# MartinPippel/DAmar

Hardware: AMD Instinct MI355X
Metric: aligned base-pairs/sec (daligner block-vs-block) (higher is better)
Workload: dtype int32

## Files before the change

damar_amd/csrc/kernels/kernels.h:

```cpp
#ifndef DAMAR_KERNELS_H
#define DAMAR_KERNELS_H

#include "dev_common.h"

size_t damar_scan_workspace_bytes(u64 n);
void   damar_exclusive_scan_u32(const u32 *in, u32 *out, u64 n, void *work, u64 *total_dev, hipStream_t st);
#define DAMAR_SCAN_TILE 4096
void   damar_tile_offsets_u32(const u32 *in, u64 n, void *work, u64 *total_dev, hipStream_t st);
void   damar_scan_tile_counts(u32 *tcount, u32 ntiles, u64 *total_dev, hipStream_t st);
size_t damar_sort_workspace_bytes(u64 n);
void   damar_sort_set_threads(int threads);
const u32 *damar_sort_error_word(const void *work);
int    damar_radix_sort_keys_u64(u64 *k0, u64 *k1, u64 n, int lobit, int hibit, void *work, hipStream_t st);
void   damar_radix_sort_split_u64(u64 *k0, u64 *k1, u64 n, int lobit, int hibit, u32 *ohi, u32 *olo, void *work,
                                  hipStream_t st);
int    damar_radix_sort_u32(u32 *k0, u32 *v0, u32 *k1, u32 *v1, u64 n, int nbits, void *work, hipStream_t st);
int    damar_radix_sort_keys_u32(u32 *k0, u32 *k1, u64 n, int nbits, void *work, hipStream_t st);
int    damar_radix_sort_u64(u64 *k0, u32 *v0, u64 *k1, u32 *v1, u64 n, int nbits, void *work, hipStream_t st);

enum { DAMAR_PILE_COVER = 0, DAMAR_PILE_REPEAT = 1, DAMAR_PILE_TANDEM = 2 };
#define DAMAR_PILE_ERR_RANGE 1u
typedef struct
{
  const long long *pile_off;
  const int *pile_aread, *abpos, *aepos, *bbpos, *bepos, *bread, *flags, *read_len, *read_flags;
  u32   npiles;
  int   mode, pbits;
  int   min_len, inc_identity, inccov, enter, leave, merge_dist;
  u64  *keys;
  u32  *kept;
  const u32 *koff;
  u64  *bases;
  int  *active;
  int  *rb, *re, *rc;
  int  *out;
  u32  *count;
  u64  *stats;
  u32  *err;
} PileArgs;
void damar_launch_pile_events(const PileArgs *a, hipStream_t st);
void damar_launch_pile_sweep(const PileArgs *a, hipStream_t st);
void damar_launch_pile_gather(const int *out, const u32 *koff, const u32 *count, const u32 *doff, u32 npiles, int *dst, hipStream_t st);

typedef struct
{ const u8  *bases;
  const u32 *pk;
  u32        rbias;
  const u32 *boff;
  const u32 *coarse;
  u32        nreads;
  u32        total;
  int        maxlen;
  int        rpbits;
  const u32 *moff;
  const int *mdat;
} DevBlock;

#define SEED_PRIO_VAR(name, dflt) static __device__ int name = dflt;  static int name##_host = dflt;
#define SEED_PRIO(name)     do { if (name) __builtin_amdgcn_s_setprio(3); } while (0)
#define SEED_PRIO_SETTER(fn, name) \
  void fn(int on) { if (on != name##_host) { HIP_CHECK(hipMemcpyToSymbol(HIP_SYMBOL(name), &on, sizeof(int)));  name##_host = on; } }

#define COARSE_SHIFT 9
#define PK_PAD 4

#ifdef __HIPCC__
__device__ __forceinline__ u32 read_of_pos(const DevBlock &b, u32 p)
{ u32 r = b.coarse[p >> COARSE_SHIFT];
  while (b.boff[r + 1] <= p)
    r += 1;
  return r;
}
__device__ __forceinline__ void pos_decode(const DevBlock &b, u32 v, u32 *r, u32 *x)
{ if (b.rpbits)
    { *r = v >> b.rpbits;
      *x = v & ((1u << b.rpbits) - 1u);
    }
  else
    { const u32 rr = read_of_pos(b, v);
      *r = rr;
      *x = v - b.boff[rr];
    }
}
__device__ __forceinline__ u32 pos_encode(const DevBlock &b, u32 r, u32 x, u32 p)
{ return b.rpbits ? ((r << b.rpbits) | x) : p; }
#endif

long long damar_pack_words(u32 total);
void damar_launch_pack_bases(const u8 *bases, u32 total, u32 *pk, hipStream_t st);
void damar_launch_unpack_bps(const u8 *raw, const u32 *foff, const DevBlock *blk, int comp, u8 *bases, hipStream_t st);

void damar_preload_index(void);  void damar_preload_scan(void);  void damar_preload_sort(void);
void damar_preload_merge(void);  void damar_preload_report(void);
void damar_sort_set_prio(int on);
void damar_merge_set_prio(int on);
void damar_index_set_prio(int on);
void damar_launch_kmer_tuples(const DevBlock *blk, int kmer, u32 nkmers, void *codes, int wide, u32 *pos, hipStream_t st);
void damar_launch_mask_flags(const DevBlock *blk, int kmer, const u32 *pos, u32 n, u32 *keep, hipStream_t st);
void damar_launch_biased_tuples(const DevBlock *blk, int kmer, const int *logbase, void *codes, int wide, u32 *pos,
                                u32 *keep, hipStream_t st);
void damar_launch_suppress_flags(const void *codes, int wide, u32 n, int suppress, u32 *keep, hipStream_t st);
void damar_launch_compact_pairs(const void *k, int wide, const u32 *v, const u32 *keep, const u32 *off, u32 n,
                                void *ko, u32 *vo, hipStream_t st);

void damar_launch_tandem_links(const DevBlock *blk, int kmer, const void *codes, int wide, const u32 *pos, u32 n,
                               int *dist, hipStream_t st);

typedef struct
{ const void *acode;  const u32 *apos;  u32 alen;
  const void *bcode;  const u32 *bpos;  u32 blen;
  int  wide;
  int  kbits;
  int  self, comp, identity;
  u32  limit;
  DevBlock ablk, bblk;
  int  pbits, abits;
  int  dbits;
  u32  b_lo, b_hi;
} MergeArgs;

typedef struct { u32 b0, b1, ja, ia;
                 u32 sh, pad[3]; } MergeTile;

size_t damar_merge_workspace_bytes(u32 alen);
u32   *damar_merge_tile_counts(void *work, u32 alen);
u32    damar_merge_tiles(u32 alen);
void   damar_launch_merge_count(const MergeArgs *m, void *work, unsigned long long *gram, u32 ngram, hipStream_t st);
void damar_launch_merge_emit(const MergeArgs *m, void *work, u64 nhits, u64 *keys, u32 *vals, u32 *pid, hipStream_t st);
void damar_launch_merge_bread_hist(const MergeArgs *m, void *work, unsigned long long *hist, hipStream_t st);
void damar_launch_merge_range(const MergeArgs *m, void *work, hipStream_t st);
void damar_launch_pair_heads_ids(const u32 *pids, u64 nhits, u64 off, u64 gtotal, int abits, int minhit, int nshift,
                                 u64 *send, u64 *bits, void *scan_work, u64 *total_dev, u32 *heads, hipStream_t st);
void damar_launch_pair_bitmap(const u32 *pids, const u32 *heads, u32 nheads, int abits, u32 b_lo, u32 b_hi, u32 *bitmap,
                              hipStream_t st);
void damar_launch_seed_cut_count(const u64 *keys, u64 nhits, int pbits, const u32 *bitmap, u32 *tcount, u64 *total_dev,
                                 hipStream_t st);
void damar_launch_seed_cut_scatter(const u64 *keys, const u32 *vals, u64 nhits, int pbits, const u32 *bitmap,
                                   const u32 *toff, u64 *okeys, u32 *ovals, hipStream_t st);
// ... 174 lines not shown
```

damar_amd/csrc/kernels/kmer_index.hip:

```cpp
#include "dev_common.h"
#include "kernels.h"

SEED_PRIO_VAR(g_index_prio, 0)
SEED_PRIO_SETTER(damar_index_set_prio, g_index_prio)


template <typename CodeT, bool PACK>
__global__ __launch_bounds__(256)
void kmer_tuples(DevBlock blk, int kmer, u32 nkmers, CodeT *__restrict__ codes, u32 *__restrict__ pos)
{ SEED_PRIO(g_index_prio);
  const u32 p = blockIdx.x * 256u + threadIdx.x;
  if (p >= blk.total)
    return;
  const u32 r = read_of_pos(blk, p), b0 = blk.boff[r];
  if (p - b0 < (u32) (kmer - 1) || p + 1 == blk.boff[r + 1])
    return;
  const u32 i = p - (r + 1) * (u32) kmer + 1;
  if (i >= nkmers)
    return;
  CodeT c = 0;
  if (PACK)
    {
      const u32 f = p - (u32) (kmer - 1), wq = f >> 4, o = (f & 15) << 1;
      u64 win = ((u64) blk.pk[wq + 1] << 32) | (u64) blk.pk[wq];
      win >>= o;
      u64 r = __brevll(win);
      r = ((r >> 1) & 0x5555555555555555ull) | ((r & 0x5555555555555555ull) << 1);
      c = (CodeT) (r >> (64 - 2 * kmer));
    }
  else
    { const u8 *s = blk.bases + (p - (u32) (kmer - 1));
      for (int j = 0; j < kmer; j++)
        c = (CodeT) (c << 2) | (CodeT) s[j];
    }
  const u32 pw = pos_encode(blk, r, p - b0, p);
  if (PACK)
    codes[i] = (CodeT) ((u64) c << 32) | (CodeT) pw;
  else
    { codes[i] = c;
      pos[i]   = pw;
    }
}

void damar_launch_kmer_tuples(const DevBlock *blk, int kmer, u32 nkmers, void *codes, int wide, u32 *pos, hipStream_t st)
{ if (nkmers == 0)
    return;
  if (wide)
    hipLaunchKernelGGL((kmer_tuples<u64, false>), dim3((blk->total + 255) / 256), dim3(256), 0, st, *blk, kmer, nkmers, (u64 *) codes, pos);
  else if (pos == NULL)
    hipLaunchKernelGGL((kmer_tuples<u64, true>), dim3((blk->total + 255) / 256), dim3(256), 0, st, *blk, kmer, nkmers, (u64 *) codes, pos);
  else
    hipLaunchKernelGGL((kmer_tuples<u32, false>), dim3((blk->total + 255) / 256), dim3(256), 0, st, *blk, kmer, nkmers, (u32 *) codes, pos);
}

__global__ __launch_bounds__(256)
void mask_flags(DevBlock blk, int kmer, const u32 *__restrict__ pos, u32 n, u32 *__restrict__ keep)
{ u32 i = blockIdx.x * 256u + threadIdx.x;
  if (i >= n)
    return;
  u32 r, x;
  pos_decode(blk, pos[i], &r, &x);
  const int e = (int) x, s = e - (kmer - 1);
  u32 lo = blk.moff[r] >> 1, hi = blk.moff[r + 1] >> 1;
  const u32 end = hi;
  while (lo < hi)
    { const u32 mid = (lo + hi) >> 1;
      if (blk.mdat[2 * mid + 1] > s) hi = mid; else lo = mid + 1;
    }
  keep[i] = (lo < end && blk.mdat[2 * lo] <= e) ? 0u : 1u;
}

void damar_launch_mask_flags(const DevBlock *blk, int kmer, const u32 *pos, u32 n, u32 *keep, hipStream_t st)
{ if (n == 0)
    return;
  hipLaunchKernelGGL(mask_flags, dim3((n + 255) / 256), dim3(256), 0, st, *blk, kmer, pos, n, keep);
}

template <typename CodeT>
__global__ __launch_bounds__(64)
void biased_tuples(DevBlock blk, int kmer, int lb0, int lb1, int lb2, int lb3,
                   CodeT *__restrict__ codes, u32 *__restrict__ pos, u32 *__restrict__ keep)
{ const u32 r = blockIdx.x * 64u + threadIdx.x;
// ... 237 lines not shown
```

damar_amd/csrc/kernels/radix_sort.hip:

```cpp
#include <atomic>
#include <type_traits>
#include "dev_common.h"
#include "kernels.h"

SEED_PRIO_VAR(g_sort_prio, 1)
SEED_PRIO_SETTER(damar_sort_set_prio, g_sort_prio)

#ifndef OS_THREADS
#define OS_THREADS 1024
#endif
#ifndef OS_MINW
#define OS_MINW    4
#endif
#ifndef OS_RANK_LDS
#define OS_RANK_LDS 1
#endif
#define OS_MINTILE (256 * 8)
#define OS_MAXPASS 8

#define OH_ITEMS   16

#define LB_COUNT   1u
#define LB_PREFIX  2u
#define LB_SPINS   (1u << 24)
#ifndef LB_AHEAD
#define LB_AHEAD   8
#endif

#define WS_HIST    256
#define WS_CTR     (256 + OS_MAXPASS * 256 * 4)
#define WS_LB      16384

template <typename GT> __device__ __forceinline__ GT lb_load(const GT *p)
{ return __hip_atomic_load(p, __ATOMIC_RELAXED, __HIP_MEMORY_SCOPE_AGENT); }
template <typename GT> __device__ __forceinline__ void lb_store(GT *p, GT v)
{ __hip_atomic_store(p, v, __ATOMIC_RELAXED, __HIP_MEMORY_SCOPE_AGENT); }

__device__ __forceinline__ u32 os_scan256(u32 v, u32 *lds4)
{ const int l = lane_id(), w = threadIdx.x >> 6;
  const u32 inc = (u32) wave_incl_scan_i((int) v);
  if (l == 63 && w < 4) lds4[w] = inc;
  __syncthreads();
  u32 base = 0;
  for (int i = 0; i < 4; i++)
    if (i < w) base += lds4[i];
  __syncthreads();
  return base + inc - v;
}


#define OH_THREADS 1024
#define OH_BINMAX  61440

template <typename KeyT>
__global__ __launch_bounds__(OH_THREADS)
void onesweep_hist(const KeyT *__restrict__ keys, u64 n, int lobit, int npass, u64 dsh ,
                   u64 dwd , u32 *__restrict__ ghist, uint4 *__restrict__ clr, u64 clr16)
{ extern __shared__ u32 sh[];
  constexpr u32 nthr = OH_THREADS;
  const int nw = npass * 128 * 32;
  for (int j = threadIdx.x; j < nw; j += nthr)
    sh[j] = 0;
  __syncthreads();
  const u32 c = threadIdx.x & 31u;
  const u64 ntile = (n + (u64) nthr * OH_ITEMS - 1) / ((u64) nthr * OH_ITEMS);
  for (u64 t = blockIdx.x; t < ntile; t += gridDim.x)
    { const u64 base = t * ((u64) nthr * OH_ITEMS);
      KeyT k[OH_ITEMS];
#pragma unroll
      for (int r = 0; r < OH_ITEMS; r++)
        { const u64 i = base + (u64) r * nthr + threadIdx.x;
          k[r] = (i < n) ? keys[i] : (KeyT) 0;
        }
#pragma unroll
      for (int r = 0; r < OH_ITEMS; r++)
        { const u64 i = base + (u64) r * nthr + threadIdx.x;
          if (i < n)
            { const KeyT x = k[r] >> lobit;
              for (int p = 0; p < npass; p++)
                { const u32 d = (u32) (x >> (int) ((dsh >> (8 * p)) & 0xffu)) & (u32) ((dwd >> (8 * p)) & 0xffu);
                  atomicAdd(&sh[((u32) p << 12) + ((d >> 1) << 5) + c], 1u << ((d & 1u) << 4));
                }
            }
        }
    }
  __syncthreads();
  for (int j = threadIdx.x; j < npass * 256; j += nthr)
    { const u32 pl = (u32) j >> 8, d = (u32) j & 0xffu, sft = (d & 1u) << 4;
      u32 sum = 0;
#pragma unroll 8
      for (u32 q = 0; q < 32; q++)
        sum += (sh[(pl << 12) + ((d >> 1) << 5) + ((q + threadIdx.x) & 31u)] >> sft) & 0xffffu;
      if (sum)
        atomicAdd(&ghist[j], sum);
    }
  const uint4 z = make_uint4(0, 0, 0, 0);
  for (u64 i = (u64) blockIdx.x * nthr + threadIdx.x; i < clr16; i += (u64) gridDim.x * nthr)
    clr[i] = z;
}

#define OH_COPIES  8
template <typename KeyT>
__global__ __launch_bounds__(256)
void onesweep_hist8(const KeyT *__restrict__ keys, u64 n, int lobit, int npass, u64 dsh ,
                   u64 dwd , u32 *__restrict__ ghist, uint4 *__restrict__ clr, u64 clr16)
{ SEED_PRIO(g_sort_prio);
  extern __shared__ u32 sh[];
  const int nb = npass * 256 * OH_COPIES;
  for (int j = threadIdx.x; j < nb; j += 256)
    sh[j] = 0;
  __syncthreads();
  const u32 c = threadIdx.x & (OH_COPIES - 1);
  const u64 ntile = (n + 256 * OH_ITEMS - 1) / (256 * OH_ITEMS);
  for (u64 t = blockIdx.x; t < ntile; t += gridDim.x)
    { const u64 base = t * (256 * OH_ITEMS);
      KeyT k[OH_ITEMS];
#pragma unroll
      for (int r = 0; r < OH_ITEMS; r++)
        { const u64 i = base + (u64) r * 256 + threadIdx.x;
          k[r] = (i < n) ? keys[i] : (KeyT) 0;
        }
#pragma unroll
      for (int r = 0; r < OH_ITEMS; r++)
        { const u64 i = base + (u64) r * 256 + threadIdx.x;
          if (i < n)
            { const KeyT x = k[r] >> lobit;
              for (int p = 0; p < npass; p++)
                { const u32 d = (u32) (x >> (int) ((dsh >> (8 * p)) & 0xffu)) & (u32) ((dwd >> (8 * p)) & 0xffu);
                  atomicAdd(&sh[(((u32) p << 8) + d) * OH_COPIES + c], 1u);
                }
            }
        }
    }
  __syncthreads();
  for (int j = threadIdx.x; j < npass * 256; j += 256)
    { u32 s = 0;
#pragma unroll
      for (int q = 0; q < OH_COPIES; q++)
        s += sh[j * OH_COPIES + q];
      if (s)
        atomicAdd(&ghist[j], s);
    }
  const uint4 z = make_uint4(0, 0, 0, 0);
  for (u64 i = (u64) blockIdx.x * 256 + threadIdx.x; i < clr16; i += (u64) gridDim.x * 256)
    clr[i] = z;
}


template <typename KeyT, typename GT, bool HV, bool SPLIT, int TH, int IT>
__global__ __launch_bounds__(TH, (IT <= 8 ? 8 : OS_MINW))
void onesweep_pass(const KeyT *__restrict__ kin, const u32 *__restrict__ vin, KeyT *__restrict__ kout,
                   u32 *__restrict__ vout, u32 *__restrict__ ohi, u64 n, int shift, u32 mask,
                   const u32 *__restrict__ ghist, GT *__restrict__ lb, GT *__restrict__ lbclear,
                   u32 *__restrict__ ctr, u32 *__restrict__ err)
{ SEED_PRIO(g_sort_prio);
  constexpr int OS_TILE = TH * IT, OS_WAVES = TH / 64, OS_WSPAN = 64 * IT;
  __shared__ __attribute__((aligned(16))) KeyT skey[OS_TILE];
  u32 *const sval = (u32 *) skey;
  typedef typename std::conditional<(OS_WAVES > 8), u16, u32>::type CntT;
  __shared__ CntT cnt[OS_WAVES][256];
  __shared__ u32  dstart[256];
  __shared__ u32  gadj[256];
  __shared__ u32  lds4[4];
  __shared__ u32  s_tile;
  constexpr int SH = (int) sizeof(GT) * 8 - 2;
  constexpr GT  VM = (((GT) 1) << SH) - 1;

  const int l = lane_id(), w = threadIdx.x >> 6;
  if (threadIdx.x == 0)
    s_tile = atomicAdd(ctr, 1u);
  for (int i = 0; i < OS_WAVES; i++)
    if (threadIdx.x < 256)
      cnt[i][threadIdx.x] = 0;
#if OS_RANK_LDS
  static_assert((size_t) OS_TILE * sizeof(KeyT) >= (size_t) OS_WAVES * 256 * sizeof(u64), "the rank words do not fit the stage");
  for (int i = threadIdx.x; i < OS_WAVES * 256; i += TH)
    ((u64 *) skey)[i] = 0;
#endif
  __syncthreads();
  const u32 tile  = (u32) __builtin_amdgcn_readfirstlane((int) s_tile);
  const u64 tbase = (u64) tile * OS_TILE;
  const u32 have = (n - tbase < (u64) OS_TILE) ? (u32) (n - tbase) : (u32) OS_TILE;
  const u32 t0 = (u32) w * OS_WSPAN + (u32) l;
  const KeyT *const tin = kin + tbase;

  KeyT key[IT];
  u32  rnk[IT];
#pragma unroll
  for (int r = 0; r < IT; r++)
    { const u32 ti = t0 + (u32) r * 64;
      key[r] = tin[ti < have ? ti : have - 1];
    }
#if OS_RANK_LDS
  u64 *const wmask = (u64 *) skey + (u32) w * 256u;
  const u64 lanebit = 1ull << l;
#pragma unroll
  for (int r = 0; r < IT; r++)
    { const bool ok = t0 + (u32) r * 64 < have;
      const u32  d  = (u32) (key[r] >> shift) & mask;
      if (ok)
        __hip_atomic_fetch_or(&wmask[d], lanebit, __ATOMIC_RELAXED, __HIP_MEMORY_SCOPE_WAVEFRONT);
      __builtin_amdgcn_fence(__ATOMIC_SEQ_CST, "wavefront");
      const u64 peers  = __hip_atomic_load(&wmask[d], __ATOMIC_RELAXED, __HIP_MEMORY_SCOPE_WAVEFRONT);
      const u32 before = cnt[w][d];
      __builtin_amdgcn_fence(__ATOMIC_SEQ_CST, "wavefront");
      const u32 mine   = __builtin_amdgcn_mbcnt_hi((u32) (peers >> 32), __builtin_amdgcn_mbcnt_lo((u32) peers, 0u));
      rnk[r] = before + mine;
      if (ok && mine == 0)
        { cnt[w][d] = (CntT) (before + (u32) __popcll(peers));
          __hip_atomic_store(&wmask[d], 0ull, __ATOMIC_RELAXED, __HIP_MEMORY_SCOPE_WAVEFRONT);
        }
      __builtin_amdgcn_fence(__ATOMIC_SEQ_CST, "wavefront");
    }
#else
#pragma unroll
  for (int r = 0; r < IT; r++)
    { const bool ok = t0 + (u32) r * 64 < have;
      const u32  d  = (u32) (key[r] >> shift) & mask;
      const u64 okm = __ballot(ok);
      u32 plo = (u32) okm, phi = (u32) (okm >> 32);
#pragma unroll
      for (int b = 0; b < 8; b++)
        { const int t  = ((int) (d << (31 - b))) >> 31;
          const u64 nm = ~__ballot(t < 0);
          plo &= (u32) nm ^ (u32) t;
          phi &= (u32) (nm >> 32) ^ (u32) t;
        }
      const u32 before = cnt[w][d];
      const u32 mine   = __builtin_amdgcn_mbcnt_hi(phi, __builtin_amdgcn_mbcnt_lo(plo, 0u));
      rnk[r] = before + mine;
      if (ok && mine == 0)
        cnt[w][d] = (CntT) (before + (u32) __popc(plo) + (u32) __popc(phi));
    }
#endif
  __syncthreads();

  u32 tot = 0;
  if (threadIdx.x < 256)
    { u32 run = 0;
#pragma unroll
      for (int i = 0; i < OS_WAVES; i++)
        { const u32 c = cnt[i][threadIdx.x];
          cnt[i][threadIdx.x] = (CntT) run;
          run += c;
// ... 77 lines not shown
        { const KeyT k = skey[i];
          const u32  d = (u32) (k >> shift) & mask;
          const u32  g = gadj[d] + i;
          if (HV) gdst[q] = g;
          if (SPLIT)
            { ohi[g]  = (u32) ((u64) k >> 32);
              vout[g] = (u32) k;
            }
          else
            kout[g] = k;
        }
    }
  if (HV)
    { const u32 *const tvin = vin + tbase;
      __syncthreads();
#pragma unroll
      for (int r = 0; r < IT; r++)
        { const u32 ti = t0 + (u32) r * 64;
          if (ti < have)
            sval[rnk[r]] = tvin[ti];
        }
      __syncthreads();
#pragma unroll
      for (int q = 0; q < IT; q++)
        { const u32 i = threadIdx.x + (u32) q * TH;
          if (i < have)
            vout[gdst[q]] = sval[i];
        }
    }
}


static int G_sort_threads = 0;

void damar_sort_set_threads(int threads) { G_sort_threads = (threads == 256 || threads == 512) ? threads : 1024; }

static int sort_threads(void)
{ if (G_sort_threads == 0)
    { const char *e = getenv("DAMAR_SORT_THREADS");
      damar_sort_set_threads(e ? atoi(e) : OS_THREADS);
    }
  return G_sort_threads;
}

size_t damar_sort_workspace_bytes(u64 n)
{ const u64 ntiles = (n + OS_MINTILE - 1) / OS_MINTILE;
  return (size_t) WS_LB + 2 * (((size_t) ntiles * 256 * sizeof(u64) + 255) & ~(size_t) 255) + 256;
}

const u32 *damar_sort_error_word(const void *work) { return (const u32 *) work; }

template <typename KeyT, typename GT, bool HV, int TH, int IT>
static void onesweep_passes(KeyT *k0, u32 *v0, KeyT *k1, u32 *v1, u64 n, int lobit, int hibit, u32 *ohi, u32 *olo,
                            char *ws, hipStream_t st)
{ constexpr int OS_TILE = TH * IT;
  const u32 ntiles = (u32) ((n + OS_TILE - 1) / OS_TILE);
  const int npass  = (hibit - lobit + 7) / 8;
  int dshift[OS_MAXPASS], dwidth[OS_MAXPASS];
  u64 dsh = 0, dwd = 0;
  { const int bits = hibit - lobit, base = bits / npass, extra = bits % npass;
    int at = 0;
    static int even = -1;
    if (even < 0)
      { const char *e = getenv("DAMAR_SORT_EVEN");
        even = e ? atoi(e) : 1;
      }
    for (int p = 0; p < npass; p++)
      { dshift[p] = at;
        dwidth[p] = even ? base + (p < extra ? 1 : 0) : (p < npass - 1 ? 8 : bits - 8 * (npass - 1));
        at += dwidth[p];
        dsh |= (u64) dshift[p] << (8 * p);
        dwd |= (u64) ((1u << dwidth[p]) - 1u) << (8 * p);
      }
  }
  const size_t region = ((size_t) ntiles * 256 * sizeof(GT) + 255) & ~(size_t) 255;
  u32 *err = (u32 *) ws, *ghist = (u32 *) (ws + WS_HIST), *ctr = (u32 *) (ws + WS_CTR);
  GT  *lbr[2] = { (GT *) (ws + WS_LB), (GT *) (ws + WS_LB + region) };
  HIP_CHECK(hipMemsetAsync(ws, 0, WS_LB, st));
  if (sort_threads() >= 512)
    { const u64 nt = (n + (u64) OH_THREADS * OH_ITEMS - 1) / ((u64) OH_THREADS * OH_ITEMS);
      const u64 maxit = OH_BINMAX / ((OH_THREADS / 32) * OH_ITEMS);
      u64 grid = nt < 512 ? nt : 512;
      if ((nt + grid - 1) / grid > maxit)
        grid = (nt + maxit - 1) / maxit;
      const size_t lds = (size_t) npass * 128 * 32 * sizeof(u32);
      {
        static std::atomic<unsigned long long> big_lds(0ull);
        int dev = 0;
        HIP_CHECK(hipGetDevice(&dev));
        const unsigned long long bit = 1ull << (dev & 63);
        if (!(big_lds.load(std::memory_order_acquire) & bit))
          { HIP_CHECK(hipFuncSetAttribute((const void *) onesweep_hist<u32>, hipFuncAttributeMaxDynamicSharedMemorySize, 8 * 16384));
            HIP_CHECK(hipFuncSetAttribute((const void *) onesweep_hist<u64>, hipFuncAttributeMaxDynamicSharedMemorySize, 8 * 16384));
            big_lds.fetch_or(bit, std::memory_order_release);
          }
      }
      hipLaunchKernelGGL(onesweep_hist<KeyT>, dim3((u32) grid), dim3(OH_THREADS), lds, st,
                         k0, n, lobit, npass, dsh, dwd, ghist, (uint4 *) lbr[0], (u64) (region / 16));
      HIP_CHECK(hipGetLastError());
    }
  else
    { const u64 nt = (n + 256 * OH_ITEMS - 1) / (256 * OH_ITEMS);
      const u32 grid = (u32) (nt < 2048 ? nt : 2048);
      hipLaunchKernelGGL(onesweep_hist8<KeyT>, dim3(grid), dim3(256), (size_t) npass * 256 * OH_COPIES * sizeof(u32), st,
                         k0, n, lobit, npass, dsh, dwd, ghist, (uint4 *) lbr[0], (u64) (region / 16));
    }
  for (int p = 0; p < npass; p++)
    { const int  side = p & 1;
      const bool last = (p == npass - 1);
      KeyT *ki = side ? k1 : k0, *ko = side ? k0 : k1;
      u32  *vi = side ? v1 : v0, *vo = side ? v0 : v1;
      const u32 mask = (1u << dwidth[p]) - 1u;
      if (last && ohi != NULL)
        hipLaunchKernelGGL((onesweep_pass<KeyT, GT, false, true, TH, IT>), dim3(ntiles), dim3(TH), 0, st,
                           ki, (const u32 *) NULL, (KeyT *) NULL, olo, ohi, n, lobit + dshift[p], mask,
                           ghist + 256 * p, lbr[side], lbr[side ^ 1], ctr + p, err);
      else
        hipLaunchKernelGGL((onesweep_pass<KeyT, GT, HV, false, TH, IT>), dim3(ntiles), dim3(TH), 0, st,
                           ki, vi, ko, vo, (u32 *) NULL, n, lobit + dshift[p], mask,
                           ghist + 256 * p, lbr[side], lbr[side ^ 1], ctr + p, err);
    }
}

template <typename KeyT, bool HV>
static int onesweep_impl(KeyT *k0, u32 *v0, KeyT *k1, u32 *v1, u64 n, int lobit, int hibit, u32 *ohi, u32 *olo,
                         void *work, hipStream_t st)
{ const int npass = (hibit - lobit + 7) / 8;
  if (n == 0 || npass <= 0)
    return 0;
  if (npass > OS_MAXPASS || n >= 0xfffffff0ull)
    { fprintf(stderr, "damar: internal error, radix sort of %llu items on %d bits\n", (unsigned long long) n, hibit - lobit);
      fflush(NULL);
      _exit(1);
    }
  const int shape = sort_threads();
  static int lb64 = -1;
  if (lb64 < 0)
    lb64 = getenv("DAMAR_SORT_LB64") != NULL;
  if (n < (1ull << 30) && !lb64)
    { if (shape == 1024)     onesweep_passes<KeyT, u32, HV, 1024, 8>(k0, v0, k1, v1, n, lobit, hibit, ohi, olo, (char *) work, st);
      else if (shape == 512) onesweep_passes<KeyT, u32, HV, 512, 16>(k0, v0, k1, v1, n, lobit, hibit, ohi, olo, (char *) work, st);
      else              onesweep_passes<KeyT, u32, HV, 256, 16>(k0, v0, k1, v1, n, lobit, hibit, ohi, olo, (char *) work, st);
    }
  else
    onesweep_passes<KeyT, u64, HV, 256, 16>(k0, v0, k1, v1, n, lobit, hibit, ohi, olo, (char *) work, st);
  return npass & 1;
}

int damar_radix_sort_u32(u32 *k0, u32 *v0, u32 *k1, u32 *v1, u64 n, int nbits, void *work, hipStream_t st)
{ return onesweep_impl<u32, true>(k0, v0, k1, v1, n, 0, nbits, NULL, NULL, work, st); }

int damar_radix_sort_keys_u32(u32 *k0, u32 *k1, u64 n, int nbits, void *work, hipStream_t st)
{ return onesweep_impl<u32, false>(k0, NULL, k1, NULL, n, 0, nbits, NULL, NULL, work, st); }

int damar_radix_sort_u64(u64 *k0, u32 *v0, u64 *k1, u32 *v1, u64 n, int nbits, void *work, hipStream_t st)
{ return onesweep_impl<u64, true>(k0, v0, k1, v1, n, 0, nbits, NULL, NULL, work, st); }

int damar_radix_sort_keys_u64(u64 *k0, u64 *k1, u64 n, int lobit, int hibit, void *work, hipStream_t st)
{ return onesweep_impl<u64, false>(k0, NULL, k1, NULL, n, lobit, hibit, NULL, NULL, work, st); }

void damar_radix_sort_split_u64(u64 *k0, u64 *k1, u64 n, int lobit, int hibit, u32 *ohi, u32 *olo, void *work,
                                hipStream_t st)
{ onesweep_impl<u64, false>(k0, NULL, k1, NULL, n, lobit, hibit, ohi, olo, work, st); }

void damar_preload_sort(void)
{ hipFuncAttributes fa;
  (void) hipFuncGetAttributes(&fa, (const void *) onesweep_hist<u64>);
}
```

damar_amd/csrc/shim.hip:

```cpp
#include <algorithm>
#include <vector>
#include <deque>
#include <string>
#include <thread>
#include <atomic>
#include <mutex>
#include <condition_variable>
#include <functional>
#include <string.h>
#include <unistd.h>

#include "kernels/dev_common.h"
#include <ctype.h>
#include "kernels/kernels.h"

extern "C" {
#include "damar_filter.h"
#include "damar_hip.h"
#include "host/damar_host.h"
}

#define MAXGRAM 10000

static void die(void)
// ... 596 lines not shown
  HIP_CHECK(hipFree(b->coarse));
  free(b);
}


struct damar_dev_index
{ size_t codes_bytes, pos_bytes;
  damar_dev_block *blk;
  int   own_block;
  void *codes;
  u32  *pos;
  u32   n;
  int   kbits, wide;
};

static u32 *H_serr = NULL;
static int  H_nserr = 0;
static void sort_verify(void)
{ for (int i = 0; i < H_nserr; i++)
    if (H_serr[i] != 0)
      { fprintf(stderr, "damar: FATAL: the radix sort's look-back timed out\n");
        die();
      }
  H_nserr = 0;
}
static void sort_check(const void *sw)
{ if (H_serr == NULL)
    HIP_CHECK(hipHostMalloc((void **) &H_serr, 64 * sizeof(u32), hipHostMallocDefault));
  if (H_nserr == 64)
    { HIP_CHECK(hipStreamSynchronize(G_st));
      sort_verify();
    }
  HIP_CHECK(hipMemcpyAsync(&H_serr[H_nserr++], damar_sort_error_word(sw), sizeof(u32), hipMemcpyDeviceToHost, G_st));
}

static bool overlap_on(void);
static bool corun_on(void);
static void pick_sort_shape(void)
{ static int forced = -1;
  if (forced < 0)
    { const char *e = getenv("DAMAR_SORT_THREADS");
      forced = e ? atoi(e) : 0;
    }
  damar_sort_set_threads(forced ? forced : 1024);
}

static int ilog2_ceil(u64 n)
{ int b = 0;
  while ((1ull << b) < n)
    b += 1;
  return b;
}

static int  B_have = 0, B_log[4];

extern "C" void damar_bias_reset(void) { B_have = 0; }

static damar_dev_index *index_build_k(damar_dev_block *blk, int own_block, int *len, int K, int suppress, int use_bias)
{ ensure_init();
  pick_sort_shape();
  if (K > 32)
    { fprintf(stderr, "damar: FATAL: -k%d: a k-mer code holds at most 32 bases\n", K);
      die();
    }
  if (blk->nreads > 0 && blk->minlen < K)
    { fprintf(stderr, "[ERROR] - daligner: Block contains reads < %dbp long !  Run DBsplit.\n", K);
      die();
    }
  int64 nk64 = (int64) blk->d.total - (int64) K * blk->nreads;
  if (nk64 <= 0)
    { *len = 0;
      if (own_block)
        damar_block_free(blk);
      return NULL;
    }
  u32 nk = (u32) nk64;
  const int kbits = 2 * K;
  const int wide = K > 16;
  const size_t cs = wide ? sizeof(u64) : sizeof(u32);
  const bool masked = blk->d.moff != NULL;
  const bool biased = use_bias != 0;
  if (biased && !B_have)
    { const double scale = -10000. / log(4.);
      for (int i = 0; i < 4; i++)
        B_log[i] = (int) ceil(scale * log((double) blk->freq[i]));
      B_have = 1;
    }
  const u32 cap = biased ? blk->d.total : nk;
  const int npass = (kbits + 7) / 8;
  damar_dev_index *ix = (damar_dev_index *) calloc(1, sizeof(damar_dev_index));
  ix->blk = blk;  ix->own_block = own_block;  ix->kbits = kbits;  ix->wide = wide;
  if (wide)
    { ix->codes = dpool_get(cs * (size_t) cap, &ix->codes_bytes);
      ix->pos   = (u32 *) dpool_get(sizeof(u32) * (size_t) cap, &ix->pos_bytes);
    }
  else
    { ix->codes = dpool_get(2 * sizeof(u32) * (size_t) cap, &ix->codes_bytes);
      ix->pos   = (u32 *) ix->codes + cap;
    }

  size_t swb = damar_sort_workspace_bytes(cap);
  arena_reserve(&G_work, pad256(sizeof(u64) * (size_t) cap) + 3 * pad256(sizeof(u32) * (size_t) cap) + pad256(swb) +
                         pad256(damar_scan_workspace_bytes(cap)) + (1 << 16));
  void *tk = arena_take(&G_work, sizeof(u64) * (size_t) cap);
  u32 *tv = (u32 *) arena_take(&G_work, sizeof(u32) * (size_t) cap);
  void *sw = arena_take(&G_work, swb);
  u32 *keep = NULL, *off = NULL;
  void *scw = NULL;
  u64 *tot = NULL;
  if (masked || biased || suppress > 0)
    { keep = (u32 *) arena_take(&G_work, sizeof(u32) * (size_t) cap);
      off  = (u32 *) arena_take(&G_work, sizeof(u32) * (size_t) cap);
      scw  = arena_take(&G_work, damar_scan_workspace_bytes(cap));
      tot  = (u64 *) arena_take(&G_work, 64);
    }

  void *k0, *k1;
  u32  *v0, *v1;
  if (wide)
    { k0 = (npass & 1) ? tk : ix->codes;  k1 = (npass & 1) ? ix->codes : tk;
      v0 = (npass & 1) ? tv : ix->pos;    v1 = (npass & 1) ? ix->pos : tv;
    }
  else
    { k0 = (npass & 1) ? tk : ix->codes;  k1 = (npass & 1) ? ix->codes : tk;
      v0 = v1 = NULL;
    }

  tick(0);
  if (biased || masked)
    {
      void *k9 = k1;
      u32  *v9 = wide ? ((v0 == tv) ? ix->pos : tv) : (u32 *) k1 + cap;
      u64   kept = 0;
      u32   nin = nk;
      if (biased)
        { nin = cap;
          HIP_CHECK(hipMemsetAsync(keep, 0, sizeof(u32) * (size_t) cap, G_st));
          damar_launch_biased_tuples(&blk->d, K, B_log, k9, wide, v9, keep, G_st);
        }
      else
        { damar_launch_kmer_tuples(&blk->d, K, nk, k9, wide, v9, G_st);
          damar_launch_mask_flags(&blk->d, K, v9, nk, keep, G_st);
        }
      damar_exclusive_scan_u32(keep, off, nin, scw, tot, G_st);
      damar_launch_compact_pairs(k9, wide, v9, keep, off, nin, k0, v0, G_st);
      HIP_CHECK(hipMemcpyAsync(&kept, tot, sizeof(u64), hipMemcpyDeviceToHost, G_st));
      HIP_CHECK(hipStreamSynchronize(G_st));
      nk = (u32) kept;
      if (nk == 0)
        { damar_index_free(ix);
          *len = 0;
          return NULL;
        }
      if (VERBOSE && biased)
        printf("\n   Revised kmer count = %u\n", nk);
    }
  else
    damar_launch_kmer_tuples(&blk->d, K, nk, k0, wide, v0, G_st);
  tick(1);
  if (wide)
    { int side = damar_radix_sort_u64((u64 *) k0, v0, (u64 *) k1, v1, nk, kbits, sw, G_st);
      if ((side ? k1 : k0) != ix->codes)
        { fprintf(stderr, "damar: internal error, sort ended on the wrong side\n");
          die();
        }
    }
  else
    damar_radix_sort_split_u64((u64 *) k0, (u64 *) k1, nk, 32, 32 + kbits, (u32 *) ix->codes, ix->pos, sw, G_st);
  sort_check(sw);
  tick(2);
  u32 n = nk;
  if (suppress > 0)
    { u64  kept = 0;
      damar_launch_suppress_flags(ix->codes, wide, n, suppress, keep, G_st);
      damar_exclusive_scan_u32(keep, off, n, scw, tot, G_st);
      damar_launch_compact_pairs(ix->codes, wide, ix->pos, keep, off, n, tk, tv, G_st);
      HIP_CHECK(hipMemcpyAsync(&kept, tot, sizeof(u64), hipMemcpyDeviceToHost, G_st));
      HIP_CHECK(hipStreamSynchronize(G_st));
      n = (u32) kept;
      HIP_CHECK(hipMemcpyAsync(ix->codes, tk, cs * (size_t) n, hipMemcpyDeviceToDevice, G_st));
      HIP_CHECK(hipMemcpyAsync(ix->pos, tv, sizeof(u32) * (size_t) n, hipMemcpyDeviceToDevice, G_st));
    }
  tick(3);
  HIP_CHECK(hipStreamSynchronize(G_st));
  sort_verify();
  G_ms[DAMAR_T_TUPLES] = lap(0, 1);
  G_ms[DAMAR_T_KSORT]  = lap(1, 2);
  G_ms[DAMAR_T_TABLE]  = lap(2, 3);
  ix->n = n;
  if (VERBOSE)
    { printf("\n   Kmer count = %u\n   Index occupies %.2fGb of HBM\n", n, ((cs + 4.) * n) / 1073741824.);
      fflush(stdout);
    }
  if (n == 0)
    { damar_index_free(ix);
      *len = 0;
      return NULL;
    }
  *len = (int) n;
  return ix;
}

extern "C" damar_dev_index *damar_index_build(damar_dev_block *blk, int own_block, int *len)
{ double t0 = now_ms();
  damar_dev_index *ix = index_build_k(blk, own_block, len, P_kmer, P_suppress, BIASED);
  H_ms[0] += now_ms() - t0;
  return ix;
}

extern "C" void damar_index_free(damar_dev_index *ix)
{ if (ix == NULL)
    return;
  HIP_CHECK(hipStreamSynchronize(G_st));
  dpool_put(ix->codes, ix->codes_bytes);
  if (ix->pos_bytes)
    dpool_put(ix->pos, ix->pos_bytes);
  if (ix->own_block)
    damar_block_free(ix->blk);
// ... 3161 lines not shown
```

include/damar_hip.h:

```cpp
#ifndef DAMAR_HIP_H
#define DAMAR_HIP_H

#include "damar_db.h"
#include "damar_align.h"

#ifdef __cplusplus
extern "C" {
#endif

int   damar_hip_init(int device);
int   damar_hip_numa_node(int device);
const char *damar_hip_device_name(void);
void  damar_hip_sync(void);
void  damar_prewarm(int gigabytes);

typedef struct damar_dev_block damar_dev_block;
damar_dev_block *damar_block_upload(const HITS_DB *block);
void damar_block_preload(const HITS_DB *block);
damar_dev_block *damar_block_upload_bg(const HITS_DB *block);
damar_dev_block *damar_block_upload_packed(const HITS_DB *block, const damar_packed *pk, int comp);
void             damar_packed_forget(const HITS_DB *block);
void             damar_block_free(damar_dev_block *blk);

typedef struct damar_dev_index damar_dev_index;
damar_dev_index *damar_index_build(damar_dev_block *blk, int own_block, int *len);
void             damar_index_free(damar_dev_index *idx);
uint64_t         damar_index_bytes(const damar_dev_index *idx);
uint64_t         damar_block_bytes(const damar_dev_block *blk);
void             damar_hbm_info(uint64_t *free_bytes, uint64_t *total_bytes);
void             damar_pool_trim(void);
void             damar_index_download(const damar_dev_index *idx, void *out);

void damar_match(const HITS_DB *ablock, const HITS_DB *bblock,
                 damar_dev_index *aidx, damar_dev_index *bidx,
                 int self, int comp, Align_Spec *spec, int64 *counts);

typedef struct
{ const HITS_DB *ablock, *bblock;
  damar_dev_index *aidx, *bidx;
  int self, comp;
  Align_Spec *spec;
  int64 counts[3];
} damar_match_job;
void damar_match_batch(damar_match_job *jobs, int njobs);

void damar_set_bread_range(int lo, int hi);

void damar_set_async(int on);
void damar_async_drain(void);
void damar_async_totals(int64 *ncheck, double *tail_ms, double *write_ms);
void damar_async_counts(int64 *seed_hits, double *report_ms, int64 *launches);
double damar_async_d2h_ms(void);
void damar_wave_totals(int64 *cells, int64 *half_steps, int64 *iterations);
void damar_write_overlaps(Align_Spec *spec, const char *dirName1, const char *dirName2,
                          const char *ablock, const char *bblock, int lastRead);

int  damar_tandem_set_params(int kmer, int binshift, int hitmin, int nthreads);
void damar_match_self(const HITS_DB *ablock, damar_dev_block *blk, Align_Spec *spec, int64 *counts);
void Match_Self(char *aname, HITS_DB *ablock, Align_Spec *settings);

int64 damar_last_seeds(void *out, int64 cap);

int  damar_last_slabs(int *b_lo , int64 *hits , int cap);
void damar_slab_totals(int64 *out );
int  damar_slab_cut(const uint64_t *hits, int nreads, uint64_t cap, int *b_lo , int64 *sums ,
                    int max_slabs);

int damar_last_limit(void);

void damar_bias_reset(void);

int damar_local_alignment_batch(damar_dev_block *ablk, damar_dev_block *bblk, int comp,
                                Align_Spec *spec, const int *tasks, int ntasks,
                                int *paths, int64 *trace_off, uint16 *traces, int64 trace_cap);

int  damar_trace_pts(damar_dev_block *ablk, int afirst, damar_dev_block *bblk, int bfirst,
                     const Overlap *ovls, int64 novl, int tbytes, int tspace, int mode, int same,
                     int64 *soff, int *diffs, int **script);
int  damar_trace_mid(damar_dev_block *ablk, int afirst, damar_dev_block *bblk, int bfirst,
                     const Overlap *ovls, int64 novl, int tbytes, int tspace, int mode, int same,
                     int64 *soff, int *diffs, int **script);
void damar_trace_last(double *ms, int64 *cnt);
void damar_trace_release(void);

// ... 67 lines not shown
```

Baseline: 50.89 billion.

## Generate k-mer keys on the fly inside radix sort histogram and first pass

Instead of materializing packed k-mer code/position tuples into a buffer and then sorting, the histogram and first onesweep pass compute each key directly from the 2-bit packed bases with a per-wave cursor that locates the read by a wave-parallel binary search over read offsets. This removes one kernel launch and a full write-and-read of the n-element u64 key array. In exchange, the histogram and first pass do extra index arithmetic and redundant packed-base loads, and the histogram kernel's access pattern changes from strided per-thread to contiguous per-wave. The k-mer code extraction is also narrowed to a 32-bit alignbit form, which only holds for k up to 16.

Result: faster. 51.95 billion (median of 6 runs) (+2.1%).

```diff
diff --git a/damar_amd/csrc/kernels/kernels.h b/damar_amd/csrc/kernels/kernels.h
--- a/damar_amd/csrc/kernels/kernels.h
+++ b/damar_amd/csrc/kernels/kernels.h
@@ -56,6 +56,10 @@
   const int *mdat;
 } DevBlock;
 
+typedef struct { DevBlock blk;  int kmer; } KmerKeys;
+void damar_radix_sort_split_kmers(const KmerKeys *src, u64 *k0, u64 *k1, u64 n, u32 *ohi, u32 *olo, void *work,
+                                  hipStream_t st);
+
 #define SEED_PRIO_VAR(name, dflt) static __device__ int name = dflt;  static int name##_host = dflt;
 #define SEED_PRIO(name)     do { if (name) __builtin_amdgcn_s_setprio(3); } while (0)
 #define SEED_PRIO_SETTER(fn, name) \
@@ -84,6 +88,46 @@
 }
 __device__ __forceinline__ u32 pos_encode(const DevBlock &b, u32 r, u32 x, u32 p)
 { return b.rpbits ? ((r << b.rpbits) | x) : p; }
+
+__device__ __forceinline__ u32 kmer_slot0(u32 b0, u32 r, int kmer) { return b0 - r * (u32) kmer; }
+
+__device__ __forceinline__ u32 kmer_code16(const u32 *__restrict__ pk, u32 f, int kmer)
+{ const u32 wq = f >> 4, o = (f & 15) << 1;
+  const u32 win = __builtin_amdgcn_alignbit(pk[wq + 1], pk[wq], o);
+  u32 r = __brev(win);
+  r = ((r >> 1) & 0x55555555u) | ((r & 0x55555555u) << 1);
+  return r >> (32 - 2 * kmer);
+}
+
+
+struct KmerCursor
+{ u32 r, ks, ke;
+
+  __device__ __forceinline__ void open(const KmerKeys &g, u32 slot)
+  { const u32 l = (u32) lane_id();
+    u32 lo = 0, hi = g.blk.nreads;
+    while (hi - lo > 1)
+      { const u32  step = (hi - lo + 63) >> 6;
+        const u32  c  = lo + l * step;
+        const bool ok = c < hi && kmer_slot0(g.blk.boff[c < hi ? c : lo], c, g.kmer) <= slot;
+        const u32  in = (u32) __popcll(wballot(ok));
+        lo += (in - 1) * step;
+        hi  = (lo + step < hi) ? lo + step : hi;
+      }
+    r  = lo;
+    ks = kmer_slot0(g.blk.boff[r], r, g.kmer);
+    ke = kmer_slot0(g.blk.boff[r + 1], r + 1, g.kmer);
+  }
+  __device__ __forceinline__ u64 key(const KmerKeys &g, u32 i)
+  { while (i >= ke)
+      { r += 1;
+        ks = ke;
+        ke = kmer_slot0(g.blk.boff[r + 1], r + 1, g.kmer);
+      }
+    const u32 f = i + r * (u32) g.kmer, x = i - ks + (u32) (g.kmer - 1);
+    return ((u64) kmer_code16(g.blk.pk, f, g.kmer) << 32) | (u64) pos_encode(g.blk, r, x, f + (u32) (g.kmer - 1));
+  }
+};
 #endif
 
 long long damar_pack_words(u32 total);
diff --git a/damar_amd/csrc/kernels/kmer_index.hip b/damar_amd/csrc/kernels/kmer_index.hip
--- a/damar_amd/csrc/kernels/kmer_index.hip
+++ b/damar_amd/csrc/kernels/kmer_index.hip
@@ -15,19 +15,12 @@
   const u32 r = read_of_pos(blk, p), b0 = blk.boff[r];
   if (p - b0 < (u32) (kmer - 1) || p + 1 == blk.boff[r + 1])
     return;
-  const u32 i = p - (r + 1) * (u32) kmer + 1;
+  const u32 i = kmer_slot0(b0, r, kmer) + (p - b0) - (u32) (kmer - 1);
   if (i >= nkmers)
     return;
   CodeT c = 0;
   if (PACK)
-    {
-      const u32 f = p - (u32) (kmer - 1), wq = f >> 4, o = (f & 15) << 1;
-      u64 win = ((u64) blk.pk[wq + 1] << 32) | (u64) blk.pk[wq];
-      win >>= o;
-      u64 r = __brevll(win);
-      r = ((r >> 1) & 0x5555555555555555ull) | ((r & 0x5555555555555555ull) << 1);
-      c = (CodeT) (r >> (64 - 2 * kmer));
-    }
+    c = (CodeT) kmer_code16(blk.pk, p - (u32) (kmer - 1), kmer);
   else
     { const u8 *s = blk.bases + (p - (u32) (kmer - 1));
       for (int j = 0; j < kmer; j++)
diff --git a/damar_amd/csrc/kernels/radix_sort.hip b/damar_amd/csrc/kernels/radix_sort.hip
--- a/damar_amd/csrc/kernels/radix_sort.hip
+++ b/damar_amd/csrc/kernels/radix_sort.hip
@@ -31,6 +31,8 @@
 #define WS_CTR     (256 + OS_MAXPASS * 256 * 4)
 #define WS_LB      16384
 
+template <typename SrcT> constexpr bool os_made = std::is_same<SrcT, KmerKeys>::value;
+
 template <typename GT> __device__ __forceinline__ GT lb_load(const GT *p)
 { return __hip_atomic_load(p, __ATOMIC_RELAXED, __HIP_MEMORY_SCOPE_AGENT); }
 template <typename GT> __device__ __forceinline__ void lb_store(GT *p, GT v)
@@ -52,9 +54,9 @@
 #define OH_THREADS 1024
 #define OH_BINMAX  61440
 
-template <typename KeyT>
+template <typename KeyT, typename SrcT = const KeyT *__restrict__>
 __global__ __launch_bounds__(OH_THREADS)
-void onesweep_hist(const KeyT *__restrict__ keys, u64 n, int lobit, int npass, u64 dsh ,
+void onesweep_hist(SrcT keys, u64 n, int lobit, int npass, u64 dsh ,
                    u64 dwd , u32 *__restrict__ ghist, uint4 *__restrict__ clr, u64 clr16)
 { extern __shared__ u32 sh[];
   constexpr u32 nthr = OH_THREADS;
@@ -66,20 +68,41 @@
   const u64 ntile = (n + (u64) nthr * OH_ITEMS - 1) / ((u64) nthr * OH_ITEMS);
   for (u64 t = blockIdx.x; t < ntile; t += gridDim.x)
     { const u64 base = t * ((u64) nthr * OH_ITEMS);
-      KeyT k[OH_ITEMS];
-#pragma unroll
-      for (int r = 0; r < OH_ITEMS; r++)
-        { const u64 i = base + (u64) r * nthr + threadIdx.x;
-          k[r] = (i < n) ? keys[i] : (KeyT) 0;
-        }
-#pragma unroll
-      for (int r = 0; r < OH_ITEMS; r++)
-        { const u64 i = base + (u64) r * nthr + threadIdx.x;
-          if (i < n)
-            { const KeyT x = k[r] >> lobit;
-              for (int p = 0; p < npass; p++)
-                { const u32 d = (u32) (x >> (int) ((dsh >> (8 * p)) & 0xffu)) & (u32) ((dwd >> (8 * p)) & 0xffu);
-                  atomicAdd(&sh[((u32) p << 12) + ((d >> 1) << 5) + c], 1u << ((d & 1u) << 4));
+      if constexpr (!os_made<SrcT>)
+        { KeyT k[OH_ITEMS];
+#pragma unroll
+          for (int r = 0; r < OH_ITEMS; r++)
+            { const u64 i = base + (u64) r * nthr + threadIdx.x;
+              k[r] = (i < n) ? keys[i] : (KeyT) 0;
+            }
+#pragma unroll
+          for (int r = 0; r < OH_ITEMS; r++)
+            { const u64 i = base + (u64) r * nthr + threadIdx.x;
+              if (i < n)
+                { const KeyT x = k[r] >> lobit;
+                  for (int p = 0; p < npass; p++)
+                    { const u32 d = (u32) (x >> (int) ((dsh >> (8 * p)) & 0xffu)) & (u32) ((dwd >> (8 * p)) & 0xffu);
+                      atomicAdd(&sh[((u32) p << 12) + ((d >> 1) << 5) + c], 1u << ((d & 1u) << 4));
+                    }
+                }
+            }
+        }
+      else
+        {
+          const u64 first = base + (u64) (threadIdx.x >> 6) * (64 * OH_ITEMS);
+          if (first < n)
+            { KmerCursor cur;
+              cur.open(keys, (u32) first);
+#pragma unroll 4
+              for (int r = 0; r < OH_ITEMS; r++)
+                { const u64 i = first + (u64) r * 64 + (threadIdx.x & 63u);
+                  if (i < n)
+                    { const KeyT x = cur.key(keys, (u32) i) >> lobit;
+                      for (int p = 0; p < npass; p++)
+                        { const u32 d = (u32) (x >> (int) ((dsh >> (8 * p)) & 0xffu)) & (u32) ((dwd >> (8 * p)) & 0xffu);
+                          atomicAdd(&sh[((u32) p << 12) + ((d >> 1) << 5) + c], 1u << ((d & 1u) << 4));
+                        }
+                    }
                 }
             }
         }
@@ -100,9 +123,9 @@
 }
 
 #define OH_COPIES  8
-template <typename KeyT>
+template <typename KeyT, typename SrcT = const KeyT *__restrict__>
 __global__ __launch_bounds__(256)
-void onesweep_hist8(const KeyT *__restrict__ keys, u64 n, int lobit, int npass, u64 dsh ,
+void onesweep_hist8(SrcT keys, u64 n, int lobit, int npass, u64 dsh ,
                    u64 dwd , u32 *__restrict__ ghist, uint4 *__restrict__ clr, u64 clr16)
 { SEED_PRIO(g_sort_prio);
   extern __shared__ u32 sh[];
@@ -114,20 +137,41 @@
   const u64 ntile = (n + 256 * OH_ITEMS - 1) / (256 * OH_ITEMS);
   for (u64 t = blockIdx.x; t < ntile; t += gridDim.x)
     { const u64 base = t * (256 * OH_ITEMS);
-      KeyT k[OH_ITEMS];
-#pragma unroll
-      for (int r = 0; r < OH_ITEMS; r++)
-        { const u64 i = base + (u64) r * 256 + threadIdx.x;
-          k[r] = (i < n) ? keys[i] : (KeyT) 0;
-        }
-#pragma unroll
-      for (int r = 0; r < OH_ITEMS; r++)
-        { const u64 i = base + (u64) r * 256 + threadIdx.x;
-          if (i < n)
-            { const KeyT x = k[r] >> lobit;
-              for (int p = 0; p < npass; p++)
-                { const u32 d = (u32) (x >> (int) ((dsh >> (8 * p)) & 0xffu)) & (u32) ((dwd >> (8 * p)) & 0xffu);
-                  atomicAdd(&sh[(((u32) p << 8) + d) * OH_COPIES + c], 1u);
+      if constexpr (!os_made<SrcT>)
+        { KeyT k[OH_ITEMS];
+#pragma unroll
+          for (int r = 0; r < OH_ITEMS; r++)
+            { const u64 i = base + (u64) r * 256 + threadIdx.x;
+              k[r] = (i < n) ? keys[i] : (KeyT) 0;
+            }
+#pragma unroll
+          for (int r = 0; r < OH_ITEMS; r++)
+            { const u64 i = base + (u64) r * 256 + threadIdx.x;
+              if (i < n)
+                { const KeyT x = k[r] >> lobit;
+                  for (int p = 0; p < npass; p++)
+                    { const u32 d = (u32) (x >> (int) ((dsh >> (8 * p)) & 0xffu)) & (u32) ((dwd >> (8 * p)) & 0xffu);
+                      atomicAdd(&sh[(((u32) p << 8) + d) * OH_COPIES + c], 1u);
+                    }
+                }
+            }
+        }
+      else
+        {
+          const u64 first = base + (u64) (threadIdx.x >> 6) * (64 * OH_ITEMS);
+          if (first < n)
+            { KmerCursor cur;
+              cur.open(keys, (u32) first);
+#pragma unroll 4
+              for (int r = 0; r < OH_ITEMS; r++)
+                { const u64 i = first + (u64) r * 64 + (threadIdx.x & 63u);
+                  if (i < n)
+                    { const KeyT x = cur.key(keys, (u32) i) >> lobit;
+                      for (int p = 0; p < npass; p++)
+                        { const u32 d = (u32) (x >> (int) ((dsh >> (8 * p)) & 0xffu)) & (u32) ((dwd >> (8 * p)) & 0xffu);
+                          atomicAdd(&sh[(((u32) p << 8) + d) * OH_COPIES + c], 1u);
+                        }
+                    }
                 }
             }
         }
@@ -147,9 +191,9 @@
 }
 
 
-template <typename KeyT, typename GT, bool HV, bool SPLIT, int TH, int IT>
+template <typename KeyT, typename GT, bool HV, bool SPLIT, int TH, int IT, typename SrcT = const KeyT *__restrict__>
 __global__ __launch_bounds__(TH, (IT <= 8 ? 8 : OS_MINW))
-void onesweep_pass(const KeyT *__restrict__ kin, const u32 *__restrict__ vin, KeyT *__restrict__ kout,
+void onesweep_pass(SrcT kin, const u32 *__restrict__ vin, KeyT *__restrict__ kout,
                    u32 *__restrict__ vout, u32 *__restrict__ ohi, u64 n, int shift, u32 mask,
                    const u32 *__restrict__ ghist, GT *__restrict__ lb, GT *__restrict__ lbclear,
                    u32 *__restrict__ ctr, u32 *__restrict__ err)
@@ -182,14 +226,28 @@
   const u64 tbase = (u64) tile * OS_TILE;
   const u32 have = (n - tbase < (u64) OS_TILE) ? (u32) (n - tbase) : (u32) OS_TILE;
   const u32 t0 = (u32) w * OS_WSPAN + (u32) l;
-  const KeyT *const tin = kin + tbase;
 
   KeyT key[IT];
   u32  rnk[IT];
-#pragma unroll
-  for (int r = 0; r < IT; r++)
-    { const u32 ti = t0 + (u32) r * 64;
-      key[r] = tin[ti < have ? ti : have - 1];
+  if constexpr (!os_made<SrcT>)
+    { const KeyT *const tin = kin + tbase;
+#pragma unroll
+      for (int r = 0; r < IT; r++)
+        { const u32 ti = t0 + (u32) r * 64;
+          key[r] = tin[ti < have ? ti : have - 1];
+        }
+    }
+  else
+    {
+      static_assert(std::is_same<KeyT, u64>::value && !HV, "made keys are packed u64 index keys");
+      const u32 wfirst = (u32) w * OS_WSPAN;
+      KmerCursor cur;
+      cur.open(kin, (u32) tbase + (wfirst < have ? wfirst : have - 1));
+#pragma unroll
+      for (int r = 0; r < IT; r++)
+        { const u32 ti = t0 + (u32) r * 64;
+          key[r] = cur.key(kin, (u32) tbase + (ti < have ? ti : have - 1));
+        }
     }
 #if OS_RANK_LDS
   u64 *const wmask = (u64 *) skey + (u32) w * 256u;
@@ -373,8 +431,10 @@
 
 template <typename KeyT, typename GT, bool HV, int TH, int IT>
 static void onesweep_passes(KeyT *k0, u32 *v0, KeyT *k1, u32 *v1, u64 n, int lobit, int hibit, u32 *ohi, u32 *olo,
-                            char *ws, hipStream_t st)
+                            char *ws, hipStream_t st, const KmerKeys *made )
 { constexpr int OS_TILE = TH * IT;
+  constexpr bool MADE = std::is_same<KeyT, u64>::value && !HV;
+  typedef const KeyT *__restrict__ KeysAt;
   const u32 ntiles = (u32) ((n + OS_TILE - 1) / OS_TILE);
   const int npass  = (hibit - lobit + 7) / 8;
   int dshift[OS_MAXPASS], dwidth[OS_MAXPASS];
@@ -413,18 +473,31 @@
         if (!(big_lds.load(std::memory_order_acquire) & bit))
           { HIP_CHECK(hipFuncSetAttribute((const void *) onesweep_hist<u32>, hipFuncAttributeMaxDynamicSharedMemorySize, 8 * 16384));
             HIP_CHECK(hipFuncSetAttribute((const void *) onesweep_hist<u64>, hipFuncAttributeMaxDynamicSharedMemorySize, 8 * 16384));
+            HIP_CHECK(hipFuncSetAttribute((const void *) onesweep_hist<u64, KmerKeys>, hipFuncAttributeMaxDynamicSharedMemorySize, 8 * 16384));
             big_lds.fetch_or(bit, std::memory_order_release);
           }
       }
-      hipLaunchKernelGGL(onesweep_hist<KeyT>, dim3((u32) grid), dim3(OH_THREADS), lds, st,
-                         k0, n, lobit, npass, dsh, dwd, ghist, (uint4 *) lbr[0], (u64) (region / 16));
+      if (made != NULL)
+        { if constexpr (MADE)
+            hipLaunchKernelGGL((onesweep_hist<KeyT, KmerKeys>), dim3((u32) grid), dim3(OH_THREADS), lds, st,
+                               *made, n, lobit, npass, dsh, dwd, ghist, (uint4 *) lbr[0], (u64) (region / 16));
+        }
+      else
+        hipLaunchKernelGGL((onesweep_hist<KeyT, KeysAt>), dim3((u32) grid), dim3(OH_THREADS), lds, st,
+                           k0, n, lobit, npass, dsh, dwd, ghist, (uint4 *) lbr[0], (u64) (region / 16));
       HIP_CHECK(hipGetLastError());
     }
   else
     { const u64 nt = (n + 256 * OH_ITEMS - 1) / (256 * OH_ITEMS);
       const u32 grid = (u32) (nt < 2048 ? nt : 2048);
-      hipLaunchKernelGGL(onesweep_hist8<KeyT>, dim3(grid), dim3(256), (size_t) npass * 256 * OH_COPIES * sizeof(u32), st,
-                         k0, n, lobit, npass, dsh, dwd, ghist, (uint4 *) lbr[0], (u64) (region / 16));
+      if (made != NULL)
+        { if constexpr (MADE)
+            hipLaunchKernelGGL((onesweep_hist8<KeyT, KmerKeys>), dim3(grid), dim3(256), (size_t) npass * 256 * OH_COPIES * sizeof(u32), st,
+                               *made, n, lobit, npass, dsh, dwd, ghist, (uint4 *) lbr[0], (u64) (region / 16));
+        }
+      else
+        hipLaunchKernelGGL((onesweep_hist8<KeyT, KeysAt>), dim3(grid), dim3(256), (size_t) npass * 256 * OH_COPIES * sizeof(u32), st,
+                           k0, n, lobit, npass, dsh, dwd, ghist, (uint4 *) lbr[0], (u64) (region / 16));
     }
   for (int p = 0; p < npass; p++)
     { const int  side = p & 1;
@@ -432,12 +505,24 @@
       KeyT *ki = side ? k1 : k0, *ko = side ? k0 : k1;
       u32  *vi = side ? v1 : v0, *vo = side ? v0 : v1;
       const u32 mask = (1u << dwidth[p]) - 1u;
-      if (last && ohi != NULL)
-        hipLaunchKernelGGL((onesweep_pass<KeyT, GT, false, true, TH, IT>), dim3(ntiles), dim3(TH), 0, st,
+      if (p == 0 && made != NULL)
+        { if constexpr (MADE)
+            { if (last && ohi != NULL)
+                hipLaunchKernelGGL((onesweep_pass<KeyT, GT, false, true, TH, IT, KmerKeys>), dim3(ntiles), dim3(TH), 0, st,
+                                   *made, (const u32 *) NULL, (KeyT *) NULL, olo, ohi, n, lobit + dshift[p], mask,
+                                   ghist + 256 * p, lbr[side], lbr[side ^ 1], ctr + p, err);
+              else
+                hipLaunchKernelGGL((onesweep_pass<KeyT, GT, false, false, TH, IT, KmerKeys>), dim3(ntiles), dim3(TH), 0, st,
+                                   *made, vi, ko, vo, (u32 *) NULL, n, lobit + dshift[p], mask,
+                                   ghist + 256 * p, lbr[side], lbr[side ^ 1], ctr + p, err);
+            }
+        }
+      else if (last && ohi != NULL)
+        hipLaunchKernelGGL((onesweep_pass<KeyT, GT, false, true, TH, IT, KeysAt>), dim3(ntiles), dim3(TH), 0, st,
                            ki, (const u32 *) NULL, (KeyT *) NULL, olo, ohi, n, lobit + dshift[p], mask,
                            ghist + 256 * p, lbr[side], lbr[side ^ 1], ctr + p, err);
       else
-        hipLaunchKernelGGL((onesweep_pass<KeyT, GT, HV, false, TH, IT>), dim3(ntiles), dim3(TH), 0, st,
+        hipLaunchKernelGGL((onesweep_pass<KeyT, GT, HV, false, TH, IT, KeysAt>), dim3(ntiles), dim3(TH), 0, st,
                            ki, vi, ko, vo, (u32 *) NULL, n, lobit + dshift[p], mask,
                            ghist + 256 * p, lbr[side], lbr[side ^ 1], ctr + p, err);
     }
@@ -445,7 +530,7 @@
 
 template <typename KeyT, bool HV>
 static int onesweep_impl(KeyT *k0, u32 *v0, KeyT *k1, u32 *v1, u64 n, int lobit, int hibit, u32 *ohi, u32 *olo,
-                         void *work, hipStream_t st)
+                         void *work, hipStream_t st, const KmerKeys *made = NULL)
 { const int npass = (hibit - lobit + 7) / 8;
   if (n == 0 || npass <= 0)
     return 0;
@@ -459,12 +544,12 @@
   if (lb64 < 0)
     lb64 = getenv("DAMAR_SORT_LB64") != NULL;
   if (n < (1ull << 30) && !lb64)
-    { if (shape == 1024)     onesweep_passes<KeyT, u32, HV, 1024, 8>(k0, v0, k1, v1, n, lobit, hibit, ohi, olo, (char *) work, st);
-      else if (shape == 512) onesweep_passes<KeyT, u32, HV, 512, 16>(k0, v0, k1, v1, n, lobit, hibit, ohi, olo, (char *) work, st);
-      else              onesweep_passes<KeyT, u32, HV, 256, 16>(k0, v0, k1, v1, n, lobit, hibit, ohi, olo, (char *) work, st);
+    { if (shape == 1024)     onesweep_passes<KeyT, u32, HV, 1024, 8>(k0, v0, k1, v1, n, lobit, hibit, ohi, olo, (char *) work, st, made);
+      else if (shape == 512) onesweep_passes<KeyT, u32, HV, 512, 16>(k0, v0, k1, v1, n, lobit, hibit, ohi, olo, (char *) work, st, made);
+      else              onesweep_passes<KeyT, u32, HV, 256, 16>(k0, v0, k1, v1, n, lobit, hibit, ohi, olo, (char *) work, st, made);
     }
   else
-    onesweep_passes<KeyT, u64, HV, 256, 16>(k0, v0, k1, v1, n, lobit, hibit, ohi, olo, (char *) work, st);
+    onesweep_passes<KeyT, u64, HV, 256, 16>(k0, v0, k1, v1, n, lobit, hibit, ohi, olo, (char *) work, st, made);
   return npass & 1;
 }
 
@@ -484,6 +569,10 @@
                                 hipStream_t st)
 { onesweep_impl<u64, false>(k0, NULL, k1, NULL, n, lobit, hibit, ohi, olo, work, st); }
 
+void damar_radix_sort_split_kmers(const KmerKeys *src, u64 *k0, u64 *k1, u64 n, u32 *ohi, u32 *olo, void *work,
+                                  hipStream_t st)
+{ onesweep_impl<u64, false>(k0, NULL, k1, NULL, n, 32, 32 + 2 * src->kmer, ohi, olo, work, st, src); }
+
 void damar_preload_sort(void)
 { hipFuncAttributes fa;
   (void) hipFuncGetAttributes(&fa, (const void *) onesweep_hist<u64>);
diff --git a/damar_amd/csrc/shim.hip b/damar_amd/csrc/shim.hip
--- a/damar_amd/csrc/shim.hip
+++ b/damar_amd/csrc/shim.hip
@@ -672,6 +672,9 @@
   return b;
 }
 
+static int  G_index_made = 0;
+extern "C" int damar_index_last_made(void) { return G_index_made; }
+
 static int  B_have = 0, B_log[4];
 
 extern "C" void damar_bias_reset(void) { B_have = 0; }
@@ -746,6 +749,14 @@
       v0 = v1 = NULL;
     }
 
+  static int gen_on = -1;
+  if (gen_on < 0)
+    { const char *e = getenv("DAMAR_INDEX_GEN");
+      gen_on = e ? atoi(e) : 1;
+    }
+  const bool made = gen_on && !wide && !masked && !biased && blk->d.rpbits > 0;
+  G_index_made = made;
+
   tick(0);
   if (biased || masked)
     {
@@ -775,7 +786,7 @@
       if (VERBOSE && biased)
         printf("\n   Revised kmer count = %u\n", nk);
     }
-  else
+  else if (!made)
     damar_launch_kmer_tuples(&blk->d, K, nk, k0, wide, v0, G_st);
   tick(1);
   if (wide)
@@ -784,6 +795,12 @@
         { fprintf(stderr, "damar: internal error, sort ended on the wrong side\n");
           die();
         }
+    }
+  else if (made)
+    { KmerKeys src;
+      src.blk  = blk->d;
+      src.kmer = K;
+      damar_radix_sort_split_kmers(&src, (u64 *) k0, (u64 *) k1, nk, (u32 *) ix->codes, ix->pos, sw, G_st);
     }
   else
     damar_radix_sort_split_u64((u64 *) k0, (u64 *) k1, nk, 32, 32 + kbits, (u32 *) ix->codes, ix->pos, sw, G_st);
diff --git a/include/damar_hip.h b/include/damar_hip.h
--- a/include/damar_hip.h
+++ b/include/damar_hip.h
@@ -30,6 +30,7 @@
 void             damar_hbm_info(uint64_t *free_bytes, uint64_t *total_bytes);
 void             damar_pool_trim(void);
 void             damar_index_download(const damar_dev_index *idx, void *out);
+int              damar_index_last_made(void);
 
 void damar_match(const HITS_DB *ablock, const HITS_DB *bblock,
                  damar_dev_index *aidx, damar_dev_index *bidx,
```
